# aalto-speech/AaltoASR

Hardware: AMD Instinct MI355X
Metric: frames/sec GMM log-lik (39-d, 50k Gauss) + MFCC, 1/2/4/8 MI355X (higher is better)
Workload: dtype f32 (2-term fp16 split on the matrix cores, f32 accumulate); 1 GPU; configs[2]: full MFCC chain (FFT -> mel -> log -> DCT -> delta/delta-delta, CMS, normalisation) + 50000-Gaussian scoring + 2-byte LNA codes on 1 h of synthetic 16 kHz audio as 360 x 10 s utterances (449280 frames), int16 samples resident in HBM; dim=39, gaussians=50000, states=3125, gpus_flag=1

## Files before the change

### aaltoasr_amd/capi.py

```python
from __future__ import annotations

import ctypes as C
import os
import re
from typing import Optional

import numpy as np

HERE = os.path.dirname(os.path.abspath(__file__))
LIB_PATH = os.path.join(os.environ.get("AASR_LIBDIR") or os.path.join(HERE, "lib"), "libaasr.so")
HEADER_PATH = os.path.join(HERE, "..", "include", "aasr.h")

AASR_OK = 0
AASR_ERR_INVALID = -1
AASR_ERR_UNSUPPORTED = -2
AASR_ERR_NO_DEVICE = -3
AASR_ERR_IO = -4
AASR_ERR_SHORT_AUDIO = -5


class AasrError(RuntimeError):
    def __init__(self, code: int, msg: str):
        super().__init__("aasr status %d: %s" % (code, msg))
        self.code = code
# ... 385 lines not shown
    def engine_layout(self, part: int = 0):
        L = lib()
        L.aasr_debug_engine_layout.argtypes = [C.c_void_p, C.c_int] + [C.c_void_p] * 5
        colmap = np.zeros(self.num_states, np.int32)
        begin = np.zeros(64, np.int32)
        real_end = np.zeros(64, np.int32)
        piv = np.zeros((64, self.dim), np.float32)
        col0 = C.c_int64(0)
        n = L.aasr_debug_engine_layout(self._h, part, _ptr(colmap), _ptr(begin), _ptr(real_end), _ptr(piv), C.byref(col0))
        if n < 0:
            return None
        return colmap, int(col0.value), begin[:n].copy(), real_end[:n].copy(), piv[:n].copy()

    def engine_plan_note(self) -> str:
        L = lib()
        L.aasr_debug_engine_plan_note.argtypes = [C.c_void_p]
        L.aasr_debug_engine_plan_note.restype = C.c_char_p
        return L.aasr_debug_engine_plan_note(self._h).decode("utf-8", "replace")

    def precision_states(self):
        a, b = C.c_int64(0), C.c_int64(0)
        check(lib().aasr_gmm_precision_states(self._h, C.byref(a), C.byref(b)))
        return int(a.value), int(b.value)

    def set_layouts(self, mask: int) -> None:
        L = lib()
        L.aasr_debug_set_layouts.argtypes = [C.c_void_p, C.c_int]
        L.aasr_debug_set_layouts.restype = None
        L.aasr_debug_set_layouts(self._h, mask)

    def own_layout(self) -> dict:
        L = lib()
        L.aasr_debug_own_layout.argtypes = [C.c_void_p, C.POINTER(C.c_int64)]
        L.aasr_debug_own_layout.restype = None
        out = (C.c_int64 * 6)()
        L.aasr_debug_own_layout(self._h, out)
        return {"two_term_rows": bool(out[0]), "routing": bool(out[1]), "outlier_comps": int(out[2]),
                "outlier_states": int(out[3]), "all_centred": bool(out[4]), "probe_moved": int(out[5])}

    def outlier_path(self):
        L = lib()
        L.aasr_debug_outlier_path.argtypes = [C.c_void_p, C.POINTER(C.c_int64)]
        L.aasr_debug_outlier_path.restype = None
        out = (C.c_int64 * 2)()
        L.aasr_debug_outlier_path(self._h, out)
        return int(out[0]), int(out[1])

    def set_outlier_fuse(self, on: bool) -> None:
        L = lib()
        L.aasr_debug_set_outlier_fuse.argtypes = [C.c_void_p, C.c_int]
        L.aasr_debug_set_outlier_fuse.restype = None
        L.aasr_debug_set_outlier_fuse(self._h, 1 if on else 0)

    def active_layout(self) -> int:
        L = lib()
        L.aasr_debug_active_layout.argtypes = [C.c_void_p]
        return L.aasr_debug_active_layout(self._h)

    def _check_frames(self, frames) -> None:
        if frames.ndim != 2 or frames.shape[1] != self.dim:
            raise ValueError("frames must be [F x %d], got %s" % (self.dim, tuple(frames.shape)))

    def score(self, frames: np.ndarray) -> np.ndarray:
        frames = np.ascontiguousarray(frames, np.float32)
        self._check_frames(frames)
        out = np.empty((frames.shape[0], self.num_states), np.float32)
        check(lib().aasr_gmm_score(self._h, _ptr(frames), frames.shape[0], _ptr(out)))
        return out

    def score_dev(self, d_frames, d_out, stream=None) -> None:
        check(lib().aasr_gmm_score_dev(self._h, _ptr(d_frames), d_frames.shape[0], _ptr(d_out),
                                       _stream_handle(stream)))

    def score_scratch_floats(self, F: int) -> int:
        return lib().aasr_gmm_score_scratch_floats(self._h, F)

    def score_lna_dev(self, d_frames, d_scratch, d_bytes, normalize: bool = True, lnabytes: int = 2, stream=None) -> None:
        check(lib().aasr_gmm_score_lna_dev(self._h, d_frames.data_ptr(), d_frames.shape[0], int(normalize), lnabytes,
                                           d_scratch.data_ptr(), d_bytes.data_ptr(), _stream_handle(stream)))

    def score_pitch_ok(self) -> bool:
        return bool(lib().aasr_gmm_score_pitch_ok(self._h))

    def score_dev_pitched(self, d_frames, d_out, pitch: int, stream=None) -> None:
        check(lib().aasr_gmm_score_dev_pitched(self._h, _ptr(d_frames), d_frames.shape[0], _ptr(d_out),
                                               pitch, _stream_handle(stream)))

    def gauss_loglik(self, frames: np.ndarray) -> np.ndarray:
        frames = np.ascontiguousarray(frames, np.float32)
        self._check_frames(frames)
        out = np.empty((frames.shape[0], self.num_gaussians), np.float32)
        check(lib().aasr_gmm_gauss_loglik(self._h, _ptr(frames), frames.shape[0], _ptr(out)))
        return out


def lna_encode(state_loglik: np.ndarray, normalize: bool = True, lnabytes: int = 2):
    x = np.ascontiguousarray(state_loglik, np.float32)
    F, S = x.shape
    lp = np.empty((F, S), np.float32)
    by = np.empty((F, S * lnabytes), np.uint8)
    check(lib().aasr_lna_encode(_ptr(x), F, S, int(normalize), lnabytes, _ptr(lp), _ptr(by)))
    return lp, by


def lna_encode_dev(d_loglik, normalize: bool, lnabytes: int, d_lp=None, d_bytes=None, stream=None,
                   num_states: Optional[int] = None):
# ... 542 lines not shown
```

### aaltoasr_amd/csrc/gmm.h

```cpp
#pragma once
#include <cmath>
#include <cstdint>
#include <string>
#include <functional>
#include <memory>
#include <vector>

#include "common.h"

namespace aasr {

struct HostModel {
  int dim = 0;
  int64_t G = 0;
  std::vector<double> mean, var;
  std::vector<double> cov;
  std::vector<uint8_t> is_full;
  bool any_full() const { return !is_full.empty(); }
  std::vector<double> gauss_bias;
  int n_transforms = 0;
  std::vector<int32_t> g2t;
  std::vector<double> xform;
  double logw_bias = 0;
  double logw(size_t k) const {
// ... 204 lines not shown
    int64_t cols = 0;
    int arith = 0;
    int64_t states = 0;
  };
  std::vector<EnginePart> engine_parts;
  std::string engine_plan_note;
  aasr::DevBuf<int32_t> engine_colmap;
  std::vector<int32_t> engine_colmap_h;
  int64_t engine_cols = 0;
  bool is_engine_part = false;
  mutable aasr::DevBuf<float> engine_scratch, engine_part_scratch;
  std::vector<uint8_t> f16_state_ok;
  int64_t f16_probe_moved = 0;
  bool f16_whole_rejected = false;
  aasr::FullLayout full;
  int num_cus = 0;
  int layout_mask = 7;
  bool use_bf16x3 = true;
  double kappa_matrix = 0, kappa2_matrix = 0;
  bool centred_ok = false, ill_conditioned = false;
  double kappa = 0;
  int centred_dimp = 0;
  aasr::DevBuf<float> centred_recs;
  aasr::DevBuf<int32_t> centred_state_off;
  aasr::DevBuf<int32_t> centred_splits;
  int centred_max_splits = 1;
  bool f64_built = false;
  int f64_dimp = 0;
  aasr::DevBuf<double> f64_recs, f64_x, f64_out, f64_A, f64_b, f64_xframes;
  double f64_det = 1.0;
  aasr::DevBuf<int32_t> f64_state_off;
  int f64_classes = 0;
  aasr::DevBuf<int32_t> f64_rec_class;
  aasr::DevBuf<double> f64_class_A, f64_class_b, f64_class_det, f64_class_x;
  bool pool_centred_built = false;
  aasr::DevBuf<float> poolc_recs;
  aasr::DevBuf<int32_t> poolc_state_off, poolc_splits;
  int poolc_max_splits = 1;
  std::vector<uint8_t> outlier;
  bool hyb_enabled = false;
  int64_t hyb_states = 0, hyb_rows = 0;
  aasr::DevBuf<float> hyb_recs;
  aasr::DevBuf<int32_t> hyb_state_off;
  aasr::DevBuf<int32_t> hyb_splits;
  int hyb_max_splits = 1;
  aasr::DevBuf<int32_t> hyb_map;
  std::vector<int32_t> hyb_comps;
  std::vector<int32_t> parent_gauss;
  aasr::DevBuf<float> hyb_scratch;
  aasr::DevBuf<uint32_t> hyb_tab;
  mutable struct HybFuse { const float *part = nullptr; int64_t pitch = 0; bool used = false; } hyb_fuse;
  mutable int64_t hyb_fused_launches = 0, hyb_merge_passes = 0;
  bool hyb_fuse_off = false;
  bool rows_unbiased = false;
  double out_bias_ln = 0;
  bool class_routing = false;
  std::vector<int32_t> class_g2t;
  std::vector<std::unique_ptr<aasr_gmm>> dim_parts;
  std::vector<int32_t> dim_part_off;
  aasr::DevBuf<float> dim_part_x, dim_part_ll;
  aasr::DevBuf<int32_t> dim_mix_off, dim_mix_idx;
  aasr::DevBuf<float> dim_mix_logw;
  std::unique_ptr<aasr_gmm> pool_view;
  std::vector<std::unique_ptr<aasr_gmm>> class_models;
  std::vector<aasr::DevBuf<double>> class_a, class_b;
  std::vector<double> class_logdet;
  aasr::DevBuf<float> class_scratch, class_xframes;
  std::shared_ptr<void> utt_scratch;
  std::shared_ptr<void> recipe_scratch;
  aasr::DevBuf<double> xf_a, xf_b;
  aasr::DevBuf<float> d_xframes;
  aasr::ClusterState cl;
  aasr::DevBuf<float> d_frames, d_out;
  mutable aasr::DevBuf<uint32_t> fop_scratch;
};

namespace aasr {
void gmm_build(aasr_gmm *g, const HostModel &m);
void gmm_set_transforms(aasr_gmm *g, int32_t n_transforms, const int32_t *gauss_to_transform, const double *W);
void gmm_build_pool(aasr_gmm *g);
void gmm_dim_split_score(aasr_gmm *g, const float *d_frames, int64_t F, float *d_out, bool per_gaussian, hipStream_t stream,
                         const unsigned long long *maskw = nullptr, int c1 = 0, const int32_t *gclus = nullptr,
                         bool frames_adapted = false);
void gmm_build_pool_centred(aasr_gmm *g);
void gmm_build_f64(aasr_gmm *g);
void gmm_cluster_score_f64_launch(aasr_gmm *g, const double *d_frames, const double *d_members, int64_t F,
                                  double *d_out, int linear, double det, hipStream_t stream);
void gmm_f64_masked_launch(aasr_gmm *g, const double *d_members, int64_t F, double *d_out, int linear, double det,
                           const int32_t *crow, const unsigned long long *maskw, int c1, const double *ll64,
                           int64_t Cs, int C, hipStream_t stream);
void gmm_f64_classes_masked_launch(aasr_gmm *g, const double *d_frames, int64_t n, double *d_out, int linear,
                                   const int32_t *crow, const unsigned long long *maskw, int c1, const double *ll64,
                                   int64_t Cs, int C, hipStream_t stream);
void gmm_score_f64_launch(aasr_gmm *g, const double *d_frames, int64_t F, double *d_out, int linear,
                          hipStream_t stream);
void gmm_build_tracks(aasr_gmm *g, bool grouped);
void gmm_probe_f16x2(aasr_gmm *g);
void gmm_plan_engine_parts(aasr_gmm *g);
bool gmm_engine_parts_active(const aasr_gmm *g);
bool gmm_engine_parts_clustered(const aasr_gmm *g);
void gmm_scatter_columns(const float *dense, int64_t F, int64_t n, float *out, int64_t pitch, hipStream_t stream);
void gmm_add_bias_nofloor(float *d_out, int64_t n, float bias, hipStream_t stream);
void gmm_gather_engine_columns(const aasr_gmm *g, const float *rows, int64_t F, int64_t in_pitch, float *out, int64_t out_pitch,
                               hipStream_t stream);
int64_t gmm_engine_pitch(const aasr_gmm *g);
int64_t gmm_engine_pitch_max(const aasr_gmm *g);
// ... 37 lines not shown
```

### aaltoasr_amd/csrc/gmm_score.hip

```cpp
#include <hip/hip_runtime.h>
#include <mutex>
#include <unordered_map>

#include <cmath>
#include <cstdlib>

#include "gmm.h"

namespace aasr {

typedef float f32x16 __attribute__((ext_vector_type(16)));
typedef float f32x4 __attribute__((ext_vector_type(4)));
typedef float f32x2 __attribute__((ext_vector_type(2)));

#define LN2_F 0.69314718055994530942f
#define LOG2E_F 1.4426950408889634074f
#define LOG_TINY_F (-115.12925464970228f)
#define NEG_BIG_F (-3.0e38f)
#ifndef AASR_ABLATION
#define AASR_ABLATION 0
#endif
#if AASR_ABLATION
#define AASR_DBG(bits) (dbg & (bits))
#else
// ... 868 lines not shown

struct PivotGroups {
  const int32_t *colend = nullptr;
  int64_t fop_stride = 0;
  const float *pivots = nullptr;
  const float *tabs = nullptr;
  int sc = 0;
  const uint32_t *hyb_tab = nullptr;
  const float *hyb_part = nullptr;
  int64_t hyb_pitch = 0;
  float hyb_bias = 0.0f;
};

template <int NK16, bool GROUPED, bool WIDE, int NS>
struct PlSmem {
  static constexpr int kTileBytes = NK16 * NS * 2 * 64 * 16;
  static constexpr int NBUF = WIDE ? 3 : 2;
  static constexpr bool kBig = WIDE && GROUPED && NBUF * kTileBytes + 8 * FRAMES_PER_WAVE * 34 * 4 <= 160 * 1024;
  static constexpr int OG = kBig ? 32 : 16;
  static constexpr int kOutStride = kBig ? 34 : 20;
  static constexpr int kOutFloatsPerWave = GROUPED ? FRAMES_PER_WAVE * kOutStride : 0;
  static constexpr int kMapBytes = NBUF * 16 * 4;
  static constexpr int kBytes = NBUF * kTileBytes + (WIDE ? 8 : 4) * kOutFloatsPerWave * 4 + kMapBytes;
};

constexpr int kMapCol = 0xffffff;
constexpr int kMapEmpty = 1 << 28;
constexpr int kMapFlush16 = 1 << 29;
constexpr int kMapFlush32 = 1 << 30;

#ifdef AASR_PL_TRACE
__device__ unsigned long long g_pl_trace[8][12];
#ifndef AASR_PL_TRACE_BLOCK
#define AASR_PL_TRACE_BLOCK 300
#endif
#define PL_TRACE_DECL unsigned long long tr_tiles = 0, tr_sub[3] = {0, 0, 0}, tr_acc[8] = {0, 0, 0, 0, 0, 0, 0, 0}, tr_prev = __builtin_readcyclecounter(), tr_t0 = tr_prev, tr_bar = 0, tr_vm = 0
#define PL_TRACE(k) do { const unsigned long long tr_now = __builtin_readcyclecounter(); tr_acc[k] += tr_now - tr_prev; tr_prev = tr_now; } while (0)
#else
#define PL_TRACE_DECL
#define PL_TRACE(k)
#endif
#ifndef AASR_PL_PRIO
#define AASR_PL_PRIO 1
#endif
#ifndef AASR_PL_PRIO_SCHEME
#define AASR_PL_PRIO_SCHEME 1
#endif
#ifndef AASR_PL_PRIO_HI
#define AASR_PL_PRIO_HI 2
#endif
#ifndef AASR_PL_PRIO_LO
#define AASR_PL_PRIO_LO 1
#endif
template <int NK16, bool GROUPED, bool CL, bool WIDE, int NS, bool MAPPED = false, bool PGF = false, bool HYB = false>
__global__ __launch_bounds__(WIDE ? 512 : 256, WIDE ? 1 : 2) void k_gmm_diag_score_pl(
    const float *__restrict__ frames, int64_t F, int dim, const float *__restrict__ pivot,
    const uint16_t *__restrict__ apack, const int32_t *__restrict__ split_row,
    const uint16_t *__restrict__ close_mask, const int32_t *__restrict__ sid, int sid_stride,
    float *__restrict__ out, int64_t S, int64_t pitch, float ref_ln, int dbg, ClusterArgs cl,
    const u32x4 *__restrict__ fop, CutPlan plan, PivotGroups pg) {
  extern __shared__ __attribute__((aligned(16))) char smem_raw[];
  typedef PlSmem<NK16, GROUPED, WIDE, NS> SM;
  int blk, cut;
  if ((int)blockIdx.x < plan.n_main) {
    cut = (int)blockIdx.x / plan.blocks_main;
    blk = (int)blockIdx.x - cut * plan.blocks_main;
  } else {
    const int b = (int)blockIdx.x - plan.n_main;
    cut = b / plan.blocks_rem;
    blk = plan.blocks_main + (b - cut * plan.blocks_rem);
    split_row = plan.split_rem;
  }
  blk = __builtin_amdgcn_readfirstlane(blk);
  cut = __builtin_amdgcn_readfirstlane(cut);
  PL_TRACE_DECL;
  constexpr int OG = SM::OG;
  constexpr int kTileFloats = SM::kTileBytes / 4;
  constexpr int kOS = SM::kOutStride;
  constexpr int NW = WIDE ? 8 : 4;
  constexpr int NPROD = NS * (NS + 1) / 2;
  constexpr int MPH = NK16 * NPROD * 2;
  float *abuf0 = (float *)smem_raw;
  const int tid = threadIdx.x;
  const int wave = tid >> 6;
  const int lane = tid & 63;
  constexpr int NBUF = SM::NBUF;
  float *ost = abuf0 + NBUF * kTileFloats + wave * SM::kOutFloatsPerWave;
  int *emap = (int *)(abuf0 + NBUF * kTileFloats + NW * SM::kOutFloatsPerWave);
#ifndef AASR_PL_SADDR_COPY
#define AASR_PL_SADDR_COPY 1
#endif
  const unsigned lane_off16 = (unsigned)lane * 16u;
  auto issue_tile = [&](int64_t tile, int b) {
    if (AASR_PL_SADDR_COPY) {
      constexpr int kChunks = kTileFloats / 4 / 64;
      const char *gbase = (const char *)((const float *)apack + (size_t)tile * kTileFloats);
      const unsigned lbase = (unsigned)__builtin_amdgcn_readfirstlane((int)(unsigned)(uintptr_t)(abuf0 + b * kTileFloats));
#ifndef AASR_PL_COPY_IMM
#define AASR_PL_COPY_IMM 1
#endif
      constexpr int kRounds = (kChunks + NW - 1) / NW;
      if (AASR_PL_COPY_IMM && kRounds <= 4) {
        const int w = __builtin_amdgcn_readfirstlane(wave);
        const int c0 = w * kRounds;
        const unsigned long long sb = (unsigned long long)(uintptr_t)gbase + (unsigned long long)c0 * 1024ull;
        const unsigned lo = (unsigned)__builtin_amdgcn_readfirstlane((int)(unsigned)sb);
        const unsigned hi = (unsigned)__builtin_amdgcn_readfirstlane((int)(unsigned)(sb >> 32));
        const unsigned long long sbase = (unsigned long long)lo | ((unsigned long long)hi << 32);
        const unsigned dst = (unsigned)__builtin_amdgcn_readfirstlane((int)(lbase + (unsigned)c0 * 1024u));
        const int cnt = kChunks - c0 < kRounds ? kChunks - c0 : kRounds;
        if (cnt >= 4)
          asm volatile("s_mov_b32 m0, %0\n\tglobal_load_lds_dwordx4 %1, %2\n\tglobal_load_lds_dwordx4 %1, %2 offset:1024\n\t"
                       "global_load_lds_dwordx4 %1, %2 offset:2048\n\tglobal_load_lds_dwordx4 %1, %2 offset:3072"
                       : : "s"(dst), "v"(lane_off16), "s"(sbase) : "memory", "m0");
        else if (cnt == 3)
          asm volatile("s_mov_b32 m0, %0\n\tglobal_load_lds_dwordx4 %1, %2\n\tglobal_load_lds_dwordx4 %1, %2 offset:1024\n\t"
                       "global_load_lds_dwordx4 %1, %2 offset:2048"
                       : : "s"(dst), "v"(lane_off16), "s"(sbase) : "memory", "m0");
        else if (cnt == 2)
          asm volatile("s_mov_b32 m0, %0\n\tglobal_load_lds_dwordx4 %1, %2\n\tglobal_load_lds_dwordx4 %1, %2 offset:1024"
                       : : "s"(dst), "v"(lane_off16), "s"(sbase) : "memory", "m0");
        else if (cnt == 1)
          asm volatile("s_mov_b32 m0, %0\n\tglobal_load_lds_dwordx4 %1, %2" : : "s"(dst), "v"(lane_off16), "s"(sbase) : "memory", "m0");
      } else {
#pragma unroll
      for (int k = 0; k < (kChunks + NW - 1) / NW; k++) {
        const int c = __builtin_amdgcn_readfirstlane(wave) + k * NW;
        if (c < kChunks) {
          const unsigned long long sb = (unsigned long long)(uintptr_t)gbase + (unsigned long long)c * 1024ull;
          const unsigned lo = (unsigned)__builtin_amdgcn_readfirstlane((int)(unsigned)sb);
          const unsigned hi = (unsigned)__builtin_amdgcn_readfirstlane((int)(unsigned)(sb >> 32));
          const unsigned long long sbase = (unsigned long long)lo | ((unsigned long long)hi << 32);
          const unsigned dst = (unsigned)__builtin_amdgcn_readfirstlane((int)(lbase + (unsigned)c * 1024u));
          asm volatile("s_mov_b32 m0, %0\n\tglobal_load_lds_dwordx4 %1, %2" : : "s"(dst), "v"(lane_off16), "s"(sbase) : "memory", "m0");
        }
      }
      }
    } else {
      issue_tile_copy_raw((const float *)apack + (size_t)tile * kTileFloats, abuf0 + b * kTileFloats, kTileFloats, wave, lane, NW);
    }
    if (MAPPED && wave == NW - 1 && lane < 16) {
      const int32_t *src = sid + tile * 16 + lane;
      const unsigned dst = (unsigned)__builtin_amdgcn_readfirstlane((int)(unsigned)(uintptr_t)(emap + b * 16));
      asm volatile("s_mov_b32 m0, %0\n\tglobal_load_lds_dword %1, off" : : "s"(dst), "v"(src) : "memory", "m0");
    }
  };
#ifdef AASR_PL_NOLAG
  const int group = 0;
#else
  const int group = WIDE ? __builtin_amdgcn_readfirstlane(wave >> 2) : 0;
#endif
  auto matrix_prio = [&](int phase) {
    if (AASR_PL_PRIO_SCHEME >= 1 && WIDE) {
      const bool hi = AASR_PL_PRIO_SCHEME == 1 ? ((group == 1) == (phase == 1)) : ((group == 1) != (phase == 1));
      if (hi) __builtin_amdgcn_s_setprio(AASR_PL_PRIO_HI);
      else __builtin_amdgcn_s_setprio(AASR_PL_PRIO_LO);
    } else if (AASR_PL_PRIO > 0) {
      __builtin_amdgcn_s_setprio(AASR_PL_PRIO);
    }
  };
#ifdef AASR_PL_JB
  constexpr int JB = AASR_PL_JB < NK16 ? AASR_PL_JB : 0;
#else
  constexpr int JB = 0;
#endif
  const int n = lane & 31;
  const int h = lane >> 5;
  const int64_t f0 = (int64_t)blk * (NW * FRAMES_PER_WAVE) + wave * FRAMES_PER_WAVE;

  const int64_t t_begin = split_row[4 * cut];
  const int64_t t_end = split_row[4 * cut + 4];
  if (t_begin < t_end) issue_tile(t_begin, 0);
  if (t_begin + 1 < t_end) issue_tile(t_begin + 1, 1);
  int pgi = 0;
  if (pg.colend) {
    pgi = split_row[4 * cut + 3];
    if (!PGF) fop += (size_t)pgi * pg.fop_stride;
    S = pg.colend[pgi];
  }

  u32x4 bq[NK16][NS][2];
  if constexpr (PGF && NS == 2) {
    const float *pv = pg.pivots + (size_t)pgi * dim;
    const float *tab = pg.tabs + (size_t)pgi * (3 * 8 * NK16);
#pragma unroll
    for (int nb = 0; nb < 2; nb++) {
      int64_t f = f0 + nb * 32 + n;
      if (f > F - 1) f = F - 1;
      const float *xr = frames + f * dim;
#pragma unroll
      for (int j = 0; j < NK16; j++) {
        unsigned w1[4], w2[4];
        fop_unit_f16(xr, dim, pv, tab, 8 * NK16, j, h, pg.sc, w1, w2);
        bq[j][0][nb] = u32x4{w1[0], w1[1], w1[2], w1[3]};
        bq[j][1][nb] = u32x4{w2[0], w2[1], w2[2], w2[3]};
      }
    }
  } else {
    const u32x4 *bw = fop + ((size_t)blk * NW + wave) * (NK16 * NS * 2 * 64) + lane;
#pragma unroll
    for (int j = 0; j < NK16; j++)
#pragma unroll
      for (int sp = 0; sp < NS; sp++)
#pragma unroll
        for (int nb = 0; nb < 2; nb++) bq[j][sp][nb] = bw[((j * NS + sp) * 2 + nb) * 64];
  }

  asm volatile("s_waitcnt vmcnt(0)" ::: "memory");
  __syncthreads();

  PL_TRACE(6);
  float s0 = 0.0f, s1 = 0.0f;
  int closes = split_row[4 * cut + 1 + (GROUPED ? 0 : h)];
  int hyb_st = 0x7fffffff;
  float hyb_v0 = LOG_TINY_F, hyb_v1 = LOG_TINY_F;
  uint32_t hyb_e_next = 0xffffu;
  uint32_t hyb_pend = 0xffffu;
  auto hyb_issue = [&](uint32_t e) {
    hyb_st = 0x7fffffff;
    hyb_e_next = 0xffffu;
    if ((e & 0xffffu) != 0xffffu) {
      hyb_st = (int)(e & 0xffffu);
      const float *pr = pg.hyb_part + (int64_t)(e >> 16) * pg.hyb_pitch;
      const int64_t fa = f0 + n < F ? f0 + n : F - 1, fb = f0 + 32 + n < F ? f0 + 32 + n : F - 1;
      hyb_v0 = pr[fa];
      hyb_v1 = pr[fb];
// ... 85 lines not shown
          }
        } else {
          const int pairs_closed = closes;
          if constexpr (HYB) {
            const int stc = 2 * (pairs_closed - 1) + h;
            if ((hyb_pend & 0xffffu) != 0xffffu && stc == (int)(hyb_pend & 0xffffu)) {
              hyb_issue(hyb_pend);
              hyb_pend = 0xffffu;
            }
            if (stc == hyb_st) {
              l0 = merge_floored_shares(l0, fmaxf(hyb_v0 + pg.hyb_bias, LOG_TINY_F));
              l1 = merge_floored_shares(l1, fmaxf(hyb_v1 + pg.hyb_bias, LOG_TINY_F));
              hyb_pend = hyb_e_next;
              hyb_st = 0x7fffffff;
            }
          }
          const int slot = ((2 * (pairs_closed - 1)) & (OG - 1)) + h;
          ost[n * kOS + slot] = l0;
          ost[(32 + n) * kOS + slot] = l1;
          const int64_t closed = 2 * (int64_t)pairs_closed < S ? 2 * (int64_t)pairs_closed : S;
          if (((2 * pairs_closed) & (OG - 1)) == 0 || 2 * (int64_t)pairs_closed >= S) {
            const int64_t s_base = ((closed - 1) / OG) * OG;
            flush_group(s_base, (int)(closed - s_base));
          }
        }
      }
    }
  };

  float t0 = 0.0f, t1 = 0.0f;
  auto epi_step = [&](int k, int mb, const f32x16 &c0, const f32x16 &c1, unsigned long long bits, float (&P)[2][4]) {
    const int nb = k >> 4, q = (k >> 2) & 3, e = k & 3;
    float v = nb ? c1[4 * q + e] : c0[4 * q + e];
    if (CL) v = mask_select(v, bits, 32 * nb + 8 * q + 4 * mb + e);
    float x;
    if (AASR_DBG(64)) asm volatile("v_mov_b32 %0, %1" : "=v"(x) : "v"(v));
    else asm volatile("v_exp_f32 %0, %1\n\ts_nop 0" : "=v"(x) : "v"(v));
    if (e == 0) t0 = x;
    else if (e == 1) asm volatile("v_add_f32 %0, %1, %2" : "=v"(t0) : "v"(t0), "v"(x));
    else if (e == 2) t1 = x;
    else {
      asm volatile("v_add_f32 %0, %1, %2" : "=v"(t1) : "v"(t1), "v"(x));
      asm volatile("v_add_f32 %0, %1, %2" : "=v"(P[nb][q]) : "v"(t0), "v"(t1));
    }
  };

  u32x4 afr[2][NS];
  auto load_frags = [&](const float *tile, int j, int mb, int set) {
    const u32x4 *afrag = (const u32x4 *)tile + lane;
#pragma unroll
    for (int sp = NS - 1; sp >= 0; sp--) afr[set][sp] = afrag[((j * NS + sp) * 2 + mb) * 64];
  };

  int lane_zero = 0;
  asm volatile("" : "+v"(lane_zero));
  f32x16 cA0 = {0}, cA1 = {0}, cB0 = {0}, cB1 = {0};
  unsigned long long bits_cur = 0, bits_prev = 0;
  unsigned mask_cur = 0, mask_prev = 0;
  unsigned mask_v = 0;
  if (t_begin < t_end) {
    mask_cur = (unsigned)__builtin_amdgcn_readfirstlane((int)close_mask[t_begin]);
    if (CL) bits_cur = mrow[(size_t)t_begin * TILE_ROWS];
    load_frags(abuf0, 0, 0, 0);
  }
  int bi = 0;
  int ep0[4] = {0, 0, 0, 0}, ep1[4] = {0, 0, 0, 0};
  for (int64_t t = t_begin; t < t_end; t++) {
    float *acur = abuf0 + bi * kTileFloats;
    const int bn = bi + 1 < NBUF ? bi + 1 : 0, bnn = bn + 1 < NBUF ? bn + 1 : 0;
    float *anext = abuf0 + bn * kTileFloats;
    const int bcur = bi;
    bi = bn;
    auto tile_barrier = [&]() {
#ifdef AASR_PL_TRACE
      const unsigned long long tb0 = __builtin_readcyclecounter();
#endif
      asm volatile("s_waitcnt vmcnt(0)" : "+v"(mask_v) : : "memory");
#ifdef AASR_PL_TRACE
      const unsigned long long tb1 = __builtin_readcyclecounter();
      tr_vm += tb1 - tb0;
#endif
      if (!AASR_DBG(16)) __builtin_amdgcn_s_barrier();
#ifdef AASR_PL_TRACE
      const unsigned long long tb2 = __builtin_readcyclecounter();
      tr_acc[5] += tb2 - tb1;
#endif
      if (t + 2 < t_end) issue_tile(t + 2, bnn);
      if constexpr (HYB) {
        if ((hyb_pend & 0xffffu) != 0xffffu) {
          hyb_issue(hyb_pend);
          hyb_pend = 0xffffu;
        }
      }
#ifdef AASR_PL_TRACE
      tr_bar += __builtin_readcyclecounter() - tb0;
#endif
    };
    mask_v = ((const uint32_t *)close_mask)[((t + 1) >> 1) + lane_zero];
    unsigned long long bits_next = 0;
    if (CL && t + 1 < t_end) bits_next = mrow[(size_t)(t + 1) * TILE_ROWS];
    int en00[4] = {0, 0, 0, 0}, en01[4] = {0, 0, 0, 0}, en10[4] = {0, 0, 0, 0}, en11[4] = {0, 0, 0, 0};
    if (MAPPED) {
      const int ev = emap[bcur * 16 + (lane & 15)];
#pragma unroll
      for (int q = 0; q < 4; q++) {
        en00[q] = __builtin_amdgcn_readlane(ev, q);
// ... 90 lines not shown
#endif
    if (!WIDE || group == 0) tile_barrier();
    else asm volatile("" : "+v"(mask_v));
#ifdef AASR_PL_TRACE
    const unsigned long long ts0 = __builtin_readcyclecounter();
#endif
    if (t + 1 < t_end) {
      load_frags(anext, 0, 0, 0);
      __builtin_amdgcn_sched_barrier(0);
    }
#ifdef AASR_PL_TRACE
    const unsigned long long ts1 = __builtin_readcyclecounter();
    tr_sub[0] += ts1 - ts0;
#endif
    commit(P, (GROUPED ? mask_cur : (h ? mask_cur >> 8 : mask_cur)) & 0xfu, en00, en01);
#ifdef AASR_PL_TRACE
    tr_sub[1] += __builtin_readcyclecounter() - ts1;
#endif
#pragma unroll
    for (int q = 0; q < 4; q++) {
      ep0[q] = en10[q];
      ep1[q] = en11[q];
    }
    mask_prev = mask_cur;
    bits_prev = bits_cur;
    {
      const unsigned w = (unsigned)__builtin_amdgcn_readfirstlane((int)mask_v);
      mask_cur = ((t + 1) & 1) ? w >> 16 : w & 0xffffu;
    }
    bits_cur = bits_next;
  }
  if (t_begin < t_end) {
    float P[2][4];
#pragma unroll
    for (int k = 0; k < 32; k++) epi_step(k, 1, cB0, cB1, bits_prev, P);
    commit(P, (GROUPED ? mask_prev : (h ? mask_prev >> 8 : mask_prev)) >> 4 & 0xfu, ep0, ep1);
  }
#ifdef AASR_PL_TRACE
  if ((int)blockIdx.x == AASR_PL_TRACE_BLOCK && lane == 0) {
    PL_TRACE(4);
    if (WIDE && group == 1) tr_acc[0] -= tr_bar;
    else tr_acc[4] -= tr_bar;
    tr_acc[3] = tr_bar;
    tr_acc[6] = tr_vm;
    tr_acc[7] = tr_prev - tr_t0;
    for (int k = 0; k < 8; k++) g_pl_trace[wave & 7][k] = tr_acc[k];
    g_pl_trace[wave & 7][8] = tr_tiles;
    g_pl_trace[wave & 7][9] = tr_sub[0];
    g_pl_trace[wave & 7][10] = tr_sub[1];
  }
#endif
}

template <int NS>
__global__ __launch_bounds__(256) void k_frame_operand(const float *__restrict__ frames, int64_t F, int dim,
                                                       const float *__restrict__ pivot, const float *__restrict__ f16tab,
                                                       int nk16, u32x4 *__restrict__ out, int64_t n_units, int n_pg,
                                                       int64_t pg_stride, int sc) {
  const int64_t tid = (int64_t)blockIdx.x * 256 + threadIdx.x;
  const int lane = (int)(tid & 63);
  const int64_t unit = tid >> 6;
  if (unit >= n_units) return;
  const int j = (int)(unit % nk16);
  const int nb = (int)((unit / nk16) & 1);
  const int64_t blk = unit / (2 * nk16);
  const int n = lane & 31, h = lane >> 5;
  const int KH = 8 * nk16;
  int64_t f = blk * 64 + nb * 32 + n;
  if (f > F - 1) f = F - 1;
  const float *xr = frames + f * dim;
  const int k0 = 16 * j + 8 * h;
  const int d0 = sc ? 7 * j + (h ? 3 : -1) : (k0 >> 1) - 1;
  typedef float f32x4u __attribute__((ext_vector_type(4), aligned(4)));
  const bool whole = !sc && d0 >= 0 && d0 + 4 <= dim;
  float x[4];
  if (whole) {
    const f32x4u a = *(const f32x4u *)(xr + d0);
#pragma unroll
    for (int i = 0; i < 4; i++) x[i] = a[i];
  } else {
#pragma unroll
    for (int i = 0; i < 4; i++) x[i] = xr[d0 + i >= 0 && d0 + i < dim ? d0 + i : 0];
  }
  u32x4 *o = out + ((size_t)(blk * nk16 + j) * NS * 2 + nb) * 64 + lane;
  for (int g = 0; g < n_pg; g++, pivot += dim, f16tab += (NS == 2 ? 3 * KH : 0), o += pg_stride) {
    float v[8];
    if (whole) {
      const f32x4u b = *(const f32x4u *)(pivot + d0);
      f32x4u c = {0, 0, 0, 0}, e0 = {1, 1, 1, 1}, e1 = {1, 1, 1, 1};
      if (NS == 2) {
        c = *(const f32x4u *)(f16tab + 2 * KH + d0);
        e0 = *(const f32x4u *)(f16tab + k0);
        e1 = *(const f32x4u *)(f16tab + k0 + 4);
      }
#pragma unroll
      for (int i = 0; i < 4; i++) {
        const float xc = x[i] - b[i];
        float xq = xc;
        if (NS == 2) xq = fminf(fmaxf(xc, -c[i]), c[i]);
        float lin = xq, quad = xq * xq;
        if (NS == 2) {
          lin *= i < 2 ? e0[2 * i] : e1[2 * i - 4];
          quad *= i < 2 ? e0[2 * i + 1] : e1[2 * i - 3];
        }
        v[2 * i] = lin;
        v[2 * i + 1] = quad;
// ... 153 lines not shown
    attr_set[g->device & 63] = true;
  }
  const int32_t *splits_base = L.splits.p;
  const bool multi = L.n_pg > 1;
  const int cap = L.split_cap;
  const CutPlan plan = pick_cut_plan(blocks, (WIDE ? 1.0 : 2.0) * (g->num_cus > 0 ? g->num_cus : 256),
                                     L.rows_padded / TILE_ROWS, L.max_splits, 3.0, splits_base, multi ? L.n_pg : 1, cap);
  const int32_t *split_row = splits_base + (size_t)(plan.r_main - 1) * (cap + 1) * 4;
  PivotGroups pg;
  const unsigned n_items = (unsigned)(plan.n_main + (plan.r_rem ? plan.blocks_rem * plan.r_rem : 0));
  if constexpr (GROUPED && NS == 2) {
    static const int pgf_env = AASR_EXPERIMENT_ENV("AASR_PGF") ? atoi(AASR_EXPERIMENT_ENV("AASR_PGF")) : 1;
    if (multi && pgf_env && L.pg_tab.p) {
      auto kern_pgf = k_gmm_diag_score_pl<NK16, GROUPED, CL, WIDE, NS, false, true>;
      static bool attr_set_pgf[64] = {false};
      if (!attr_set_pgf[g->device & 63]) {
        AASR_HIP(hipFuncSetAttribute((const void *)kern_pgf, hipFuncAttributeMaxDynamicSharedMemorySize, smem));
        attr_set_pgf[g->device & 63] = true;
      }
      pg.colend = L.pg_colend.p;
      pg.pivots = L.pg_pivot.p;
      pg.tabs = L.pg_tab.p;
      pg.sc = L.sc ? 1 : 0;
      hipLaunchKernelGGL(kern_pgf, dim3(n_items), dim3(NW * 64), smem, stream, d_frames, F,
                         g->dim, g->d_pivot.p, L.a16h.p, split_row, L.close.p, L.sid.p, L.sid_stride,
                         d_out, g->S, pitch, L.ref_ln - (float)g->out_bias_ln, dbg, cl, (const u32x4 *)nullptr, plan, pg);
      AASR_HIP(hipGetLastError());
      return;
    }
  }
  const u32x4 *fop = frame_operand<NS>(g, L, d_frames, F, blocks * NW, stream, &pg.fop_stride);
  if (multi) pg.colend = L.pg_colend.p;
  if constexpr (GROUPED && NS == 2 && !CL) {
    if (!multi && g->hyb_fuse.part && g->hyb_tab.p) {
      auto kern_hyb = k_gmm_diag_score_pl<NK16, GROUPED, CL, WIDE, NS, false, false, true>;
      static bool attr_set_hyb[64] = {false};
      if (!attr_set_hyb[g->device & 63]) {
        AASR_HIP(hipFuncSetAttribute((const void *)kern_hyb, hipFuncAttributeMaxDynamicSharedMemorySize, smem));
        attr_set_hyb[g->device & 63] = true;
      }
      pg.hyb_tab = g->hyb_tab.p;
      pg.hyb_part = g->hyb_fuse.part;
      pg.hyb_pitch = g->hyb_fuse.pitch;
      pg.hyb_bias = (float)g->out_bias_ln;
      g->hyb_fuse.used = true;
      g->hyb_fused_launches++;
      hipLaunchKernelGGL(kern_hyb, dim3(n_items), dim3(NW * 64), smem, stream, d_frames, F,
                         g->dim, g->d_pivot.p, L.a16h.p, split_row, L.close.p, L.sid.p, L.sid_stride,
                         d_out, g->S, pitch, L.ref_ln - (float)g->out_bias_ln, dbg, cl, fop, plan, pg);
      AASR_HIP(hipGetLastError());
      return;
    }
  }
  hipLaunchKernelGGL(kern, dim3(n_items), dim3(NW * 64), smem, stream, d_frames, F,
                     g->dim, g->d_pivot.p, NS == 3 ? L.a16.p : L.a16h.p, split_row, L.close.p,
                     L.sid.p, L.sid_stride,
                     d_out, g->S, pitch, L.ref_ln - (float)g->out_bias_ln, dbg, cl, fop, plan, pg);
  AASR_HIP(hipGetLastError());
}

template <int N, int NS>
static constexpr bool wide_ok() {
  if (NS == 2) return PlSmem<N, true, true, NS>::kBytes <= 160 * 1024;
  return 3 * Bf16Smem<N, true, true, NS>::kTileBytes + 8 * Bf16Smem<N, true, true, NS>::kOutFloatsPerWave * 4 <= 160 * 1024 &&
         PlSmem<N, true, true, NS>::kBytes <= 160 * 1024;
}

template <int NS>
static bool launch_split(const aasr_gmm *g, const TrackLayout &L, const float *d_frames, int64_t F,
                         float *d_out, hipStream_t stream, const ClusterArgs *cl = nullptr, int64_t pitch = 0) {
  if (pitch <= 0) pitch = g->S;
  if (NS == 3 ? !L.a16.p : !L.a16h.p) return false;
  const bool grouped = L.grouped;
  const ClusterArgs none;
  static const int wide_env = AASR_EXPERIMENT_ENV("AASR_BF16_WIDE") ? atoi(AASR_EXPERIMENT_ENV("AASR_BF16_WIDE")) : -1;
  const int wide = wide_env >= 0 ? wide_env : (F >= 8192 ? 1 : 0);
  switch (L.nk16) {
#define AASR_LAUNCH(N, GR, CLF, WD, CLA)                                                   \
  do {                                                                                     \
    if constexpr (NS == 2 || (AASR_PL_BF16X3 && N <= 5))                                   \
      launch_pl_t<N, GR, CLF, WD, NS>(g, L, d_frames, F, d_out, stream, CLA, pitch);        \
    else if (L.n_pg > 1) {                                                                  \
       \
      if constexpr (GR) launch_pl_t<N, true, CLF, WD, NS>(g, L, d_frames, F, d_out, stream, CLA, pitch); \
    } else                                                                                 \
      launch_bf16_t<N, GR, CLF, WD, NS>(g, L, d_frames, F, d_out, stream, CLA, pitch);      \
  } while (0)
#define AASR_CASE(N)                                                                       \
  case N:                                                                                  \
    if (cl && NS == 2 && wide && wide_ok<N, NS>()) {                                       \
       \
       \
      if constexpr (NS == 2) {                                                             \
        if (grouped) AASR_LAUNCH(N, true, true, true, *cl);                                \
        else AASR_LAUNCH(N, false, true, true, *cl);                                       \
      }                                                                                    \
    } else if (cl) {                                                                       \
      if (grouped) AASR_LAUNCH(N, true, true, false, *cl);                                 \
      else AASR_LAUNCH(N, false, true, false, *cl);                                        \
    } else if (wide && wide_ok<N, NS>()) {                                                 \
      if (grouped) AASR_LAUNCH(N, true, false, true, none);                                \
      else AASR_LAUNCH(N, false, false, true, none);                                       \
    } else {                                                                               \
      if (grouped) AASR_LAUNCH(N, true, false, false, none);                               \
      else AASR_LAUNCH(N, false, false, false, none);                                      \
    }                                                                                      \
// ... 1197 lines not shown
#undef AASR_CASE
    default:
      break;
  }
  raise(AASR_ERR_UNSUPPORTED, "no kernel instance for K/2 = %d", pr.nkk);
}

__global__ void k_affine_frames(const float *__restrict__ x, int64_t F, int dim,
                                const double *__restrict__ A, const double *__restrict__ b,
                                float *__restrict__ y) {
  int64_t idx = (int64_t)blockIdx.x * blockDim.x + threadIdx.x;
  if (idx >= F * dim) return;
  int64_t f = idx / dim;
  int i = (int)(idx - f * dim);
  double acc = b[i];
  for (int j = 0; j < dim; j++) acc += A[(size_t)i * dim + j] * (double)x[f * dim + j];
  y[idx] = (float)acc;
}

extern "C" void aasr_debug_set_layouts(aasr_gmm *g, int mask) {
  if (!g) return;
  g->layout_mask = mask;
  if ((mask & 2) && !g->tracks.ok) gmm_build_tracks(g, false);
}
extern "C" int aasr_debug_active_layout(const aasr_gmm *g) {
  if (!g) return -1;
  if ((g->layout_mask & 4) && (g->ill_conditioned || g->precision == AASR_PREC_F32_CENTRED ||
                               !(g->layout_mask & 3)) && g->centred_ok)
    return 4;
  if ((g->layout_mask & 1) && g->paired.ok) return 1;
  if ((g->layout_mask & 2) && g->tracks.ok) return 2;
  return 0;
}
extern "C" double aasr_debug_kappa(const aasr_gmm *g) { return g ? g->kappa : -1.0; }
extern "C" void aasr_debug_own_layout(const aasr_gmm *g, int64_t *out) {
  if (!g || !out) return;
  const TrackLayout &L = g->paired.ok ? g->paired : g->tracks;
  out[0] = (L.ok && L.a16h.p) ? 1 : 0;
  out[1] = g->hyb_enabled ? 1 : 0;
  out[2] = g->hyb_rows;
  out[3] = g->hyb_states;
  out[4] = g->ill_conditioned ? 1 : 0;
  out[5] = g->f16_probe_moved;
}

extern "C" void aasr_debug_outlier_path(const aasr_gmm *g, int64_t *out) {
  if (!g || !out) return;
  out[0] = g->hyb_fused_launches;
  out[1] = g->hyb_merge_passes;
}
extern "C" void aasr_debug_set_outlier_fuse(aasr_gmm *g, int on) {
  if (g) g->hyb_fuse_off = !on;
}

extern "C" int aasr_debug_engine_layout(const aasr_gmm *g, int part, int32_t *colmap, int32_t *begin, int32_t *real_end,
                                       float *pivots, int64_t *col0) {
  if (!g || part < 0 || (size_t)part >= g->engine_parts.size()) return -1;
  if (colmap) std::copy(g->engine_colmap_h.begin(), g->engine_colmap_h.end(), colmap);
  const auto &ep = g->engine_parts[(size_t)part];
  if (col0) *col0 = ep.col0;
  const aasr::HostModel &m = ep.model->host;
  const int P = m.n_pg();
  for (int p = 0; p < P; p++) {
    if (begin) begin[p] = m.pg_begin[(size_t)p];
    if (real_end) real_end[p] = m.pg_real_end[(size_t)p];
  }
  if (pivots) std::copy(m.pg_pivot.begin(), m.pg_pivot.end(), pivots);
  return P;
}
extern "C" const char *aasr_debug_engine_plan_note(const aasr_gmm *g) { return g ? g->engine_plan_note.c_str() : ""; }
extern "C" int aasr_debug_engine_parts(const aasr_gmm *g, int64_t *out, int n) {
  if (!g || !out || n < 14) return -1;
  for (int i = 0; i < n; i++) out[i] = 0;
  out[0] = (int64_t)g->engine_parts.size();
  out[1] = g->engine_cols;
  for (size_t i = 0; i < g->engine_parts.size() && i < 3; i++) {
    const auto &part = g->engine_parts[i];
    out[2 + 4 * i] = part.arith;
    out[3 + 4 * i] = part.states;
    out[4 + 4 * i] = part.arith ? part.model->paired.n_pg : 0;
    out[5 + 4 * i] = part.arith ? part.model->paired.rows_padded : (int64_t)part.model->host.mix_idx.size();
  }
  return (int)g->engine_parts.size();
}

extern "C" double aasr_debug_frame_operand_ms(aasr_gmm *g, const float *d_frames, int64_t F, int reps, void *stream_v) {
  if (!g || F <= 0 || reps <= 0) return -1.0;
  hipStream_t stream = (hipStream_t)stream_v;
  const TrackLayout &L = g->paired.ok ? g->paired : g->tracks;
  if (!L.ok || !g->use_bf16x3 || g->precision != AASR_PREC_F16X2 || !L.a16h.p || g->cl.enabled) return -1.0;
  const int NW = F >= 8192 ? 8 : 4;
  const int64_t blocks64 = (F + NW * FRAMES_PER_WAVE - 1) / (NW * FRAMES_PER_WAVE) * NW;
  hipEvent_t e0, e1;
  if (hipEventCreate(&e0) != hipSuccess || hipEventCreate(&e1) != hipSuccess) return -1.0;
  int64_t stride = 0;
  frame_operand<2>(g, L, d_frames, F, blocks64, stream, &stride);
  (void)hipEventRecord(e0, stream);
  for (int i = 0; i < reps; i++) frame_operand<2>(g, L, d_frames, F, blocks64, stream, &stride);
  (void)hipEventRecord(e1, stream);
  (void)hipEventSynchronize(e1);
  float ms = 0;
  (void)hipEventElapsedTime(&ms, e0, e1);
  (void)hipEventDestroy(e0);
  (void)hipEventDestroy(e1);
  return (double)ms / reps;
}
// ... 615 lines not shown
```

Measured before the change: 43.04 million frames/s.

## Add register-fed scoring kernel that streams A tiles directly from global memory

```diff
diff --git a/aaltoasr_amd/capi.py b/aaltoasr_amd/capi.py
--- a/aaltoasr_amd/capi.py
+++ b/aaltoasr_amd/capi.py
@@ -461,6 +461,20 @@
         L.aasr_debug_set_outlier_fuse.restype = None
         L.aasr_debug_set_outlier_fuse(self._h, 1 if on else 0)
 
+    def score_instance(self):
+        L = lib()
+        L.aasr_debug_score_instance.argtypes = [C.c_void_p, C.POINTER(C.c_int64)]
+        L.aasr_debug_score_instance.restype = None
+        out = (C.c_int64 * 2)()
+        L.aasr_debug_score_instance(self._h, out)
+        return int(out[0]), int(out[1])
+
+    def set_score_dtv(self, mode: int) -> None:
+        L = lib()
+        L.aasr_debug_set_score_dtv.argtypes = [C.c_void_p, C.c_int]
+        L.aasr_debug_set_score_dtv.restype = None
+        L.aasr_debug_set_score_dtv(self._h, mode)
+
     def active_layout(self) -> int:
         L = lib()
         L.aasr_debug_active_layout.argtypes = [C.c_void_p]
diff --git a/aaltoasr_amd/csrc/gmm.h b/aaltoasr_amd/csrc/gmm.h
--- a/aaltoasr_amd/csrc/gmm.h
+++ b/aaltoasr_amd/csrc/gmm.h
@@ -280,6 +280,8 @@
   mutable struct HybFuse { const float *part = nullptr; int64_t pitch = 0; bool used = false; } hyb_fuse;
   mutable int64_t hyb_fused_launches = 0, hyb_merge_passes = 0;
   bool hyb_fuse_off = false;
+  mutable int64_t pl_dtv_launches = 0, pl_lds_launches = 0;
+  int pl_dtv_mode = -1;
   bool rows_unbiased = false;
   double out_bias_ln = 0;
   bool class_routing = false;
diff --git a/aaltoasr_amd/csrc/gmm_score.hip b/aaltoasr_amd/csrc/gmm_score.hip
--- a/aaltoasr_amd/csrc/gmm_score.hip
+++ b/aaltoasr_amd/csrc/gmm_score.hip
@@ -944,8 +944,17 @@
 #ifndef AASR_PL_PRIO_LO
 #define AASR_PL_PRIO_LO 1
 #endif
-template <int NK16, bool GROUPED, bool CL, bool WIDE, int NS, bool MAPPED = false, bool PGF = false, bool HYB = false>
-__global__ __launch_bounds__(WIDE ? 512 : 256, WIDE ? 1 : 2) void k_gmm_diag_score_pl(
+#ifndef AASR_DTV_DEPTH
+#define AASR_DTV_DEPTH 3
+#endif
+#ifndef AASR_DTV_LAG
+#define AASR_DTV_LAG 60
+#endif
+#ifndef AASR_PL_DTV_DEFAULT
+#define AASR_PL_DTV_DEFAULT 1
+#endif
+template <int NK16, bool GROUPED, bool CL, bool WIDE, int NS, bool MAPPED, bool PGF, bool HYB, bool DTV>
+__device__ __forceinline__ void pl_score_body(
     const float *__restrict__ frames, int64_t F, int dim, const float *__restrict__ pivot,
     const uint16_t *__restrict__ apack, const int32_t *__restrict__ split_row,
     const uint16_t *__restrict__ close_mask, const int32_t *__restrict__ sid, int sid_stride,
@@ -977,7 +986,7 @@
   const int wave = tid >> 6;
   const int lane = tid & 63;
   constexpr int NBUF = SM::NBUF;
-  float *ost = abuf0 + NBUF * kTileFloats + wave * SM::kOutFloatsPerWave;
+  float *ost = abuf0 + (DTV ? 0 : NBUF * kTileFloats) + wave * SM::kOutFloatsPerWave;
   int *emap = (int *)(abuf0 + NBUF * kTileFloats + NW * SM::kOutFloatsPerWave);
 #ifndef AASR_PL_SADDR_COPY
 #define AASR_PL_SADDR_COPY 1
@@ -1062,8 +1071,8 @@
 
   const int64_t t_begin = split_row[4 * cut];
   const int64_t t_end = split_row[4 * cut + 4];
-  if (t_begin < t_end) issue_tile(t_begin, 0);
-  if (t_begin + 1 < t_end) issue_tile(t_begin + 1, 1);
+  if (!DTV && t_begin < t_end) issue_tile(t_begin, 0);
+  if (!DTV && t_begin + 1 < t_end) issue_tile(t_begin + 1, 1);
   int pgi = 0;
   if (pg.colend) {
     pgi = split_row[4 * cut + 3];
@@ -1255,6 +1264,138 @@
     for (int sp = NS - 1; sp >= 0; sp--) afr[set][sp] = afrag[((j * NS + sp) * 2 + mb) * 64];
   };
 
+  if constexpr (DTV) {
+    static_assert(!DTV || (GROUPED && !CL && NS == 2 && !MAPPED && !PGF && !HYB && (NK16 == 4 || NK16 == 5)),
+                  "the register-fed instance: grouped tracks, two terms, one pivot, unmasked, four or five slabs");
+    constexpr int DEPTH = AASR_DTV_DEPTH < NK16 ? (AASR_DTV_DEPTH < 1 ? 1 : AASR_DTV_DEPTH) : NK16 - 1;
+    constexpr int kTileVec = kTileFloats / 4;
+    u32x4 ring[NK16][NS];
+    const u32x4 *grow = (const u32x4 *)apack + lane;
+    auto ring_load = [&](int64_t tile, int j, int mb) {
+      const u32x4 *p = grow + (size_t)tile * kTileVec;
+#pragma unroll
+      for (int sp = NS - 1; sp >= 0; sp--) ring[j][sp] = p[((j * NS + sp) * 2 + mb) * 64];
+    };
+    auto ring_ahead = [&](int64_t t, int64_t tn, int s) {
+      const int a = s + DEPTH;
+      if (a < 2 * NK16) ring_load(t, a % NK16, a / NK16);
+      else ring_load(tn, a - 2 * NK16, 0);
+    };
+    int lane_zero = 0;
+    asm volatile("" : "+v"(lane_zero));
+    f32x16 cA0 = {0}, cA1 = {0}, cB0 = {0}, cB1 = {0};
+    unsigned mask_cur = 0, mask_prev = 0;
+    const int ez[4] = {0, 0, 0, 0};
+    if (t_begin < t_end) {
+      mask_cur = (unsigned)__builtin_amdgcn_readfirstlane((int)close_mask[t_begin]);
+#pragma unroll
+      for (int s = 0; s < DEPTH; s++) ring_load(t_begin, s, 0);
+    }
+    if (WIDE && group == 1 && AASR_DTV_LAG > 0) __builtin_amdgcn_s_sleep(AASR_DTV_LAG);
+    for (int64_t t = t_begin; t < t_end; t++) {
+      const int64_t tn = t + 1 < t_end ? t + 1 : t;
+      const unsigned mask_v = ((const uint32_t *)close_mask)[((t + 1) >> 1) + lane_zero];
+      float P[2][4];
+      PL_TRACE(4);
+      matrix_prio(0);
+      {
+        int mi = 0;
+#pragma unroll
+        for (int j = 0; j < NK16; j++) {
+          ring_ahead(t, tn, j);
+          __builtin_amdgcn_sched_barrier(0);
+#pragma unroll
+          for (int grp = 0; grp < NS; grp++) {
+            const int sp = NS - 1 - grp;
+#pragma unroll
+            for (int c = 0; c <= grp; c++) {
+              const int sb = grp - c;
+#pragma unroll
+              for (int nb = 0; nb < 2; nb++) {
+                if (j == 0 && grp == 0 && c == 0) {
+                  const f32x16 z = {0};
+                  if (nb == 0) cA0 = mfma_split<NS>(ring[j][sp], bq[j][sb][0], z);
+                  else cA1 = mfma_split<NS>(ring[j][sp], bq[j][sb][1], z);
+                } else {
+                  if (nb == 0) cA0 = mfma_split<NS>(ring[j][sp], bq[j][sb][0], cA0);
+                  else cA1 = mfma_split<NS>(ring[j][sp], bq[j][sb][1], cA1);
+                }
+#pragma unroll
+                for (int k = mi * 32 / MPH; k < (mi + 1) * 32 / MPH; k++) epi_step(k, 1, cB0, cB1, 0ull, P);
+                mi++;
+                __builtin_amdgcn_sched_barrier(0);
+              }
+            }
+          }
+        }
+      }
+      if (AASR_PL_PRIO > 0) __builtin_amdgcn_s_setprio(0);
+      PL_TRACE(0);
+      if (t > t_begin) commit(P, mask_prev >> 4 & 0xfu, ez, ez);
+      PL_TRACE(1);
+      matrix_prio(1);
+      {
+        int mi = 0;
+#pragma unroll
+        for (int j = 0; j < NK16; j++) {
+          ring_ahead(t, tn, NK16 + j);
+          __builtin_amdgcn_sched_barrier(0);
+#pragma unroll
+          for (int grp = 0; grp < NS; grp++) {
+            const int sp = NS - 1 - grp;
+#pragma unroll
+            for (int c = 0; c <= grp; c++) {
+              const int sb = grp - c;
+#pragma unroll
+              for (int nb = 0; nb < 2; nb++) {
+                if (j == 0 && grp == 0 && c == 0) {
+                  const f32x16 z = {0};
+                  if (nb == 0) cB0 = mfma_split<NS>(ring[j][sp], bq[j][sb][0], z);
+                  else cB1 = mfma_split<NS>(ring[j][sp], bq[j][sb][1], z);
+                } else {
+                  if (nb == 0) cB0 = mfma_split<NS>(ring[j][sp], bq[j][sb][0], cB0);
+                  else cB1 = mfma_split<NS>(ring[j][sp], bq[j][sb][1], cB1);
+                }
+#pragma unroll
+                for (int k = mi * 32 / MPH; k < (mi + 1) * 32 / MPH; k++) epi_step(k, 0, cA0, cA1, 0ull, P);
+                mi++;
+                __builtin_amdgcn_sched_barrier(0);
+              }
+            }
+          }
+        }
+      }
+      if (AASR_PL_PRIO > 0) __builtin_amdgcn_s_setprio(0);
+      PL_TRACE(2);
+#ifdef AASR_PL_TRACE
+      tr_tiles++;
+#endif
+      commit(P, mask_cur & 0xfu, ez, ez);
+      mask_prev = mask_cur;
+      {
+        const unsigned w = (unsigned)__builtin_amdgcn_readfirstlane((int)mask_v);
+        mask_cur = ((t + 1) & 1) ? w >> 16 : w & 0xffffu;
+      }
+    }
+    if (t_begin < t_end) {
+      float P[2][4];
+#pragma unroll
+      for (int k = 0; k < 32; k++) epi_step(k, 1, cB0, cB1, 0ull, P);
+      commit(P, mask_prev >> 4 & 0xfu, ez, ez);
+    }
+#ifdef AASR_PL_TRACE
+    if ((int)blockIdx.x == AASR_PL_TRACE_BLOCK && lane == 0) {
+      PL_TRACE(4);
+      tr_acc[7] = tr_prev - tr_t0;
+      for (int k = 0; k < 8; k++) g_pl_trace[wave & 7][k] = tr_acc[k];
+      g_pl_trace[wave & 7][8] = tr_tiles;
+      g_pl_trace[wave & 7][9] = 0;
+      g_pl_trace[wave & 7][10] = 0;
+    }
+#endif
+    return;
+  }
+
   int lane_zero = 0;
   asm volatile("" : "+v"(lane_zero));
   f32x16 cA0 = {0}, cA1 = {0}, cB0 = {0}, cB1 = {0};
@@ -1451,6 +1592,32 @@
 #endif
 }
 
+template <int NK16, bool GROUPED, bool CL, bool WIDE, int NS, bool MAPPED = false, bool PGF = false, bool HYB = false>
+__global__ __launch_bounds__(WIDE ? 512 : 256, WIDE ? 1 : 2) void k_gmm_diag_score_pl(
+    const float *__restrict__ frames, int64_t F, int dim, const float *__restrict__ pivot,
+    const uint16_t *__restrict__ apack, const int32_t *__restrict__ split_row,
+    const uint16_t *__restrict__ close_mask, const int32_t *__restrict__ sid, int sid_stride,
+    float *__restrict__ out, int64_t S, int64_t pitch, float ref_ln, int dbg, ClusterArgs cl,
+    const u32x4 *__restrict__ fop, CutPlan plan, PivotGroups pg) {
+  pl_score_body<NK16, GROUPED, CL, WIDE, NS, MAPPED, PGF, HYB, false>(frames, F, dim, pivot, apack, split_row, close_mask, sid,
+                                                                     sid_stride, out, S, pitch, ref_ln, dbg, cl, fop, plan, pg);
+}
+
+template <int NK16, bool WIDE>
+struct PlDtv {
+  static constexpr int kSmemBytes = (WIDE ? 8 : 4) * PlSmem<NK16, true, WIDE, 2>::kOutFloatsPerWave * 4;
+};
+template <int NK16, bool WIDE>
+__global__ __launch_bounds__(WIDE ? 512 : 256, WIDE ? 1 : 2) void k_gmm_diag_score_pl_dtv(
+    const float *__restrict__ frames, int64_t F, int dim, const float *__restrict__ pivot,
+    const uint16_t *__restrict__ apack, const int32_t *__restrict__ split_row,
+    const uint16_t *__restrict__ close_mask, const int32_t *__restrict__ sid, int sid_stride,
+    float *__restrict__ out, int64_t S, int64_t pitch, float ref_ln, int dbg, ClusterArgs cl,
+    const u32x4 *__restrict__ fop, CutPlan plan, PivotGroups pg) {
+  pl_score_body<NK16, true, false, WIDE, 2, false, false, false, true>(frames, F, dim, pivot, apack, split_row, close_mask, sid,
+                                                                       sid_stride, out, S, pitch, ref_ln, dbg, cl, fop, plan, pg);
+}
+
 template <int NS>
 __global__ __launch_bounds__(256) void k_frame_operand(const float *__restrict__ frames, int64_t F, int dim,
                                                        const float *__restrict__ pivot, const float *__restrict__ f16tab,
@@ -1710,6 +1877,26 @@
       return;
     }
   }
+  if constexpr (GROUPED && NS == 2 && !CL && (NK16 == 4 || NK16 == 5)) {
+    static const int dtv_env = AASR_EXPERIMENT_ENV("AASR_PL_DTV") ? atoi(AASR_EXPERIMENT_ENV("AASR_PL_DTV")) : -1;
+    const int want = g->pl_dtv_mode >= 0 ? g->pl_dtv_mode : dtv_env >= 0 ? dtv_env : (AASR_PL_DTV_DEFAULT && WIDE && NK16 == 5);
+    if (want && !multi) {
+      auto kern_dtv = k_gmm_diag_score_pl_dtv<NK16, WIDE>;
+      constexpr int smem_dtv = PlDtv<NK16, WIDE>::kSmemBytes;
+      static bool attr_set_dtv[64] = {false};
+      if (!attr_set_dtv[g->device & 63]) {
+        AASR_HIP(hipFuncSetAttribute((const void *)kern_dtv, hipFuncAttributeMaxDynamicSharedMemorySize, smem_dtv));
+        attr_set_dtv[g->device & 63] = true;
+      }
+      g->pl_dtv_launches++;
+      hipLaunchKernelGGL(kern_dtv, dim3(n_items), dim3(NW * 64), smem_dtv, stream, d_frames, F,
+                         g->dim, g->d_pivot.p, L.a16h.p, split_row, L.close.p, L.sid.p, L.sid_stride,
+                         d_out, g->S, pitch, L.ref_ln - (float)g->out_bias_ln, dbg, cl, fop, plan, pg);
+      AASR_HIP(hipGetLastError());
+      return;
+    }
+  }
+  g->pl_lds_launches++;
   hipLaunchKernelGGL(kern, dim3(n_items), dim3(NW * 64), smem, stream, d_frames, F,
                      g->dim, g->d_pivot.p, NS == 3 ? L.a16.p : L.a16h.p, split_row, L.close.p,
                      L.sid.p, L.sid_stride,
@@ -3013,6 +3200,17 @@
 extern "C" void aasr_debug_set_outlier_fuse(aasr_gmm *g, int on) {
   if (g) g->hyb_fuse_off = !on;
 }
+extern "C" void aasr_debug_score_instance(const aasr_gmm *g, int64_t *out) {
+  if (!g || !out) return;
+  out[0] = g->pl_dtv_launches;
+  out[1] = g->pl_lds_launches;
+}
+extern "C" void aasr_debug_set_score_dtv(aasr_gmm *g, int mode) {
+  if (g) g->pl_dtv_mode = mode < 0 ? -1 : (mode ? 1 : 0);
+}
+extern "C" int aasr_debug_score_dtv_lds_bytes(int wide) {
+  return wide ? aasr::PlDtv<5, true>::kSmemBytes : aasr::PlDtv<5, false>::kSmemBytes;
+}
 
 extern "C" int aasr_debug_engine_layout(const aasr_gmm *g, int part, int32_t *colmap, int32_t *begin, int32_t *real_end,
                                        float *pivots, int64_t *col0) {
```

Result: slower. 39.48 million frames/s (-8.3%).
